# lucidrains/progen

Hardware: NVIDIA H100
Metric: tokens_per_sec (higher is better)
Workload: dtype bf16

## Files before the change

### progen_b200/csrc/gemm_tc.cu

```cuda
#include <cuda.h>
#include <mutex>
#include <unordered_map>
#include "gemm.h"
#include "tc_ptx.cuh"

namespace {

using namespace tc;

constexpr int BM = 128;
constexpr int BN = 128;
constexpr int BK = 64;
constexpr int WG_K = 16;
constexpr int THREADS = 384;
constexpr int A_BYTES = BM * BK * 2;
constexpr int B_BYTES = BN * BK * 2;
constexpr int STAGE_BYTES = A_BYTES + B_BYTES;
constexpr int STAGES = 6;
constexpr int CS_LD = BN + 4;
constexpr int SMEM_TOTAL = 1024  + STAGES * STAGE_BYTES + 2 * STAGES * 8;
static_assert(BM * CS_LD * 4 <= STAGES * STAGE_BYTES, "the epilogue tile reuses the operand ring");
static_assert(SMEM_TOTAL <= 227 * 1024, "H100: 227 KiB of shared memory per block");

struct GemmDev {
  int M, N, K;
  int batch, batch_reduce;
  int a_batch_rows, b_batch_rows;
  long long d_batch_rows;
  int causal, split_k;
  EpiArgs epi;
};

struct TileInfo {
  int z, m0, n0, kb_begin, kb_end;
};

__device__ __forceinline__ void decode_tile(const GemmDev& g, int t, TileInfo& ti) {
  const int m_tiles = (g.M + BM - 1) / BM;
  const int n_tiles = (g.N + BN - 1) / BN;
  const int per_z = g.split_k * m_tiles * n_tiles;
  ti.z = t / per_z;
  int r = t - ti.z * per_z;
  const int ks = r / (m_tiles * n_tiles);
  r -= ks * (m_tiles * n_tiles);
  ti.m0 = (r / n_tiles) * BM;
  ti.n0 = (r % n_tiles) * BN;
  const int kb_total = (g.K + BK - 1) / BK;
  int b = 0, e = kb_total;
  if (g.causal == 1) e = min(kb_total, (ti.m0 + BM + BK - 1) / BK);
  if (g.causal == 2) b = min(kb_total, ti.m0 / BK);
  if (g.split_k > 1) {
    const int per = (kb_total + g.split_k - 1) / g.split_k;
    b = min(kb_total, ks * per);
    e = min(kb_total, b + per);
  }
  ti.kb_begin = b;
  ti.kb_end = e;
}

template <bool A_MN, bool B_MN, int KIND, typename TO>
__global__ void __launch_bounds__(THREADS, 1)
gemm_tc_kernel(const __grid_constant__ CUtensorMap tma_a, const __grid_constant__ CUtensorMap tma_b, const GemmDev g) {
  extern __shared__ uint8_t smem_raw[];
  const uint32_t raw_u32 = smem_u32(smem_raw);
  const uint32_t smem_base = (raw_u32 + 1023u) & ~1023u;
  const uint32_t bar_base = smem_base + STAGES * STAGE_BYTES;
  auto full_bar = [&](int s) { return bar_base + 8u * s; };
  auto empty_bar = [&](int s) { return bar_base + 8u * (STAGES + s); };

  const int wg = threadIdx.x >> 7;
  TileInfo ti;
  decode_tile(g, blockIdx.x, ti);

  if (threadIdx.x == 0) {
    prefetch_tensormap(&tma_a);
    prefetch_tensormap(&tma_b);
    for (int s = 0; s < STAGES; ++s) {
      mbar_init(full_bar(s), 1);
      mbar_init(empty_bar(s), 2);
    }
    fence_barrier_init();
  }
  __syncthreads();

  if (wg == 0) {
    if (threadIdx.x == 0) {
      const int a_row0 = ti.z * g.a_batch_rows;
      const int b_row0 = ti.z * g.b_batch_rows;
      int stage = 0;
      uint32_t phase = 0;
      for (int kb = ti.kb_begin; kb < ti.kb_end; ++kb) {
        mbar_wait(empty_bar(stage), phase ^ 1);
        const uint32_t sa = smem_base + stage * STAGE_BYTES;
        const uint32_t sb = sa + A_BYTES;
        mbar_expect_tx(full_bar(stage), STAGE_BYTES);
        const int k0 = kb * BK;
        if constexpr (!A_MN) {
          tma_load_2d(sa, &tma_a, full_bar(stage), k0, a_row0 + ti.m0);
        } else {
#pragma unroll
          for (int i = 0; i < BM / 64; ++i)
            tma_load_2d(sa + i * 8192, &tma_a, full_bar(stage), ti.m0 + 64 * i, a_row0 + k0);
        }
        if constexpr (!B_MN) {
          tma_load_2d(sb, &tma_b, full_bar(stage), k0, b_row0 + ti.n0);
        } else {
#pragma unroll
          for (int i = 0; i < BN / 64; ++i)
            tma_load_2d(sb + i * 8192, &tma_b, full_bar(stage), ti.n0 + 64 * i, b_row0 + k0);
        }
        if (++stage == STAGES) { stage = 0; phase ^= 1; }
      }
    }
    return;
  }

  const int c = wg - 1;
  const int t = threadIdx.x - 128;
  float acc[64];
#pragma unroll
  for (int i = 0; i < 64; ++i) acc[i] = 0.f;
  {
    int stage = 0, prev = -1;
    uint32_t phase = 0;
    for (int kb = ti.kb_begin; kb < ti.kb_end; ++kb) {
      mbar_wait(full_bar(stage), phase);
      const uint32_t sa = smem_base + stage * STAGE_BYTES;
      const uint64_t adesc = make_smem_desc<A_MN>(sa + c * 8192);
      const uint64_t bdesc = make_smem_desc<B_MN>(sa + A_BYTES);
      constexpr uint32_t a_step = A_MN ? (2048 >> 4) : (32 >> 4), b_step = B_MN ? (2048 >> 4) : (32 >> 4);
      fence_regs(acc);
      wgmma_fence();
#pragma unroll
      for (int k = 0; k < BK / WG_K; ++k)
        wgmma_m64n128k16_bf16<A_MN ? 1 : 0, B_MN ? 1 : 0>(acc, adesc + (uint64_t)(k * a_step), bdesc + (uint64_t)(k * b_step));
      wgmma_commit();
      fence_regs(acc);
      wgmma_wait<1>();
      if (prev >= 0 && (t & 127) == 0) mbar_arrive(empty_bar(prev));
      prev = stage;
      if (++stage == STAGES) { stage = 0; phase ^= 1; }
    }
    wgmma_wait<0>();
    fence_regs(acc);
  }

  asm volatile("bar.sync 1, 256;" ::: "memory");
  float* cs = reinterpret_cast<float*>(smem_raw + (smem_base - raw_u32));
  {
    const int w = (t & 127) >> 5, lane = t & 31;
    const int r0 = 64 * c + 16 * w + (lane >> 2);
    const int c0 = 2 * (lane & 3);
#pragma unroll
    for (int j = 0; j < BN / 8; ++j) {
      *reinterpret_cast<float2*>(cs + r0 * CS_LD + 8 * j + c0) = make_float2(acc[4 * j], acc[4 * j + 1]);
      *reinterpret_cast<float2*>(cs + (r0 + 8) * CS_LD + 8 * j + c0) = make_float2(acc[4 * j + 2], acc[4 * j + 3]);
    }
  }
  asm volatile("bar.sync 1, 256;" ::: "memory");

#pragma unroll 1
  for (int idx = t; idx < BM * (BN / 8); idx += 256) {
    const int r = idx / (BN / 8), cc = (idx % (BN / 8)) * 8;
    const int m = ti.m0 + r, col = ti.n0 + cc;
    if (m >= g.M || col >= g.N) continue;
    float v[8];
    const float4 x0 = *reinterpret_cast<const float4*>(cs + r * CS_LD + cc);
    const float4 x1 = *reinterpret_cast<const float4*>(cs + r * CS_LD + cc + 4);
    v[0] = x0.x; v[1] = x0.y; v[2] = x0.z; v[3] = x0.w; v[4] = x1.x; v[5] = x1.y; v[6] = x1.z; v[7] = x1.w;
    const long long row = (g.batch_reduce ? 0 : (long long)ti.z * g.d_batch_rows) + m;
    epi_apply<KIND, TO, 8>(g.epi, DirectIO{}, row, col, v, true);
  }
}

typedef CUresult (*EncodeTiledFn)(CUtensorMap*, CUtensorMapDataType, cuuint32_t, void*, const cuuint64_t*,
                                  const cuuint64_t*, const cuuint32_t*, const cuuint32_t*, CUtensorMapInterleave,
                                  CUtensorMapSwizzle, CUtensorMapL2promotion, CUtensorMapFloatOOBfill);

EncodeTiledFn get_encode_fn() {
  static EncodeTiledFn fn = nullptr;
  static std::once_flag once;
  std::call_once(once, [] {
    void* p = nullptr;
    cudaDriverEntryPointQueryResult q;
    if (cudaGetDriverEntryPoint("cuTensorMapEncodeTiled", &p, cudaEnableDefault, &q) == cudaSuccess &&
        q == cudaDriverEntryPointSuccess)
      fn = reinterpret_cast<EncodeTiledFn>(p);
  });
  return fn;
}

struct MapKey {
  const void* ptr; uint64_t inner, outer, stride; uint32_t box_inner, box_outer, elem_bytes, swizzle;
  bool operator==(const MapKey& o) const {
    return ptr == o.ptr && inner == o.inner && outer == o.outer && stride == o.stride && box_inner == o.box_inner &&
           box_outer == o.box_outer && elem_bytes == o.elem_bytes && swizzle == o.swizzle;
  }
};
struct MapKeyHash {
  size_t operator()(const MapKey& k) const {
    size_t h = std::hash<const void*>()(k.ptr);
    auto mix = [&](uint64_t v) { h ^= std::hash<uint64_t>()(v) + 0x9e3779b97f4a7c15ULL + (h << 6) + (h >> 2); };
    mix(k.inner); mix(k.outer); mix(k.stride); mix(k.box_inner); mix(k.box_outer); mix(k.elem_bytes * 256 + k.swizzle);
    return h;
  }
};

int get_tensor_map(const void* ptr, uint64_t inner, uint64_t outer, uint64_t row_stride_elems, uint32_t box_inner,
                   uint32_t box_outer, CUtensorMap* out, uint32_t elem_bytes = 2, uint32_t swizzle = 128) {
  static std::unordered_map<MapKey, CUtensorMap, MapKeyHash> cache;
  static std::mutex mu;
  MapKey key{ptr, inner, outer, row_stride_elems, box_inner, box_outer, elem_bytes, swizzle};
  std::lock_guard<std::mutex> lock(mu);
  auto it = cache.find(key);
  if (it != cache.end()) { *out = it->second; return PROGEN_OK; }
  EncodeTiledFn fn = get_encode_fn();
  if (!fn) { progen_set_error("cuTensorMapEncodeTiled driver entry point not found"); return PROGEN_ERR_DEVICE; }
  cuuint64_t dims[2] = {inner, outer};
  cuuint64_t strides[1] = {row_stride_elems * elem_bytes};
  const CUtensorMapSwizzle sw = swizzle == 128 ? CU_TENSOR_MAP_SWIZZLE_128B : swizzle == 64 ? CU_TENSOR_MAP_SWIZZLE_64B
                              : swizzle == 32 ? CU_TENSOR_MAP_SWIZZLE_32B : CU_TENSOR_MAP_SWIZZLE_NONE;
  cuuint32_t box[2] = {box_inner, box_outer};
  cuuint32_t estr[2] = {1, 1};
  CUtensorMap m;
  CUresult r = fn(&m, elem_bytes == 4 ? CU_TENSOR_MAP_DATA_TYPE_FLOAT32 : CU_TENSOR_MAP_DATA_TYPE_BFLOAT16, 2,
                  const_cast<void*>(ptr), dims, strides, box, estr, CU_TENSOR_MAP_INTERLEAVE_NONE, sw, CU_TENSOR_MAP_L2_PROMOTION_L2_256B,
                  CU_TENSOR_MAP_FLOAT_OOB_FILL_NONE);
  if (r != CUDA_SUCCESS) {
    progen_set_error("cuTensorMapEncodeTiled failed (CUresult %d) ptr=%p inner=%llu outer=%llu stride=%llu box=%ux%u", (int)r,
                     ptr, (unsigned long long)inner, (unsigned long long)outer, (unsigned long long)row_stride_elems,
                     box_inner, box_outer);
    return PROGEN_ERR_CUDA;
  }
  if (cache.size() > 4096) cache.clear();
  cache.emplace(key, m);
  *out = m;
  return PROGEN_OK;
}


template <bool A_MN, bool B_MN, int KIND, typename TO>
int launch_inst(const CUtensorMap& ta, const CUtensorMap& tb, const GemmDev& gd, int tiles, cudaStream_t stream) {
  auto kern = gemm_tc_kernel<A_MN, B_MN, KIND, TO>;
  static bool attr_set = false;
  if (!attr_set) {
    PG_CUDA(cudaFuncSetAttribute(kern, cudaFuncAttributeMaxDynamicSharedMemorySize, SMEM_TOTAL));
    attr_set = true;
  }
  kern<<<tiles, THREADS, SMEM_TOTAL, stream>>>(ta, tb, gd);
  PG_LAUNCH_CHECK();
  return PROGEN_OK;
}

}

int pg_tensor_map_2d_bf16(const void* ptr, uint64_t inner, uint64_t outer, uint64_t row_stride_elems, uint32_t box_inner,
                          uint32_t box_outer, CUtensorMap* out) {
  return get_tensor_map(ptr, inner, outer, row_stride_elems, box_inner, box_outer, out);
}

int gemm_tc_launch(const GemmArgs& a, cudaStream_t stream) {
  PG_CHECK_ARG(a.in_dtype == PG_BF16);
  PG_CHECK_ARG(a.M > 0 && a.N > 0 && a.K > 0 && a.batch >= 1 && a.split_k >= 1);
  PG_CHECK_ARG(a.N % 32 == 0);
  PG_CHECK_ARG(a.K % BK == 0);
  PG_CHECK_ARG(a.lda % 8 == 0 && a.ldb % 8 == 0);
  PG_CHECK_ARG((reinterpret_cast<uintptr_t>(a.A) & 15) == 0 && (reinterpret_cast<uintptr_t>(a.B) & 15) == 0);
  PG_CHECK_ARG(!(a.split_k > 1 && a.causal));
  if (a.epi_kind == EPI_ROTARY) PG_CHECK_ARG(a.epi.seq_len % 32 == 0);
  PG_CHECK_ARG(!(a.split_k > 1 || a.batch_reduce) || (a.epi_kind == EPI_ACCUM && a.epi.atomic));

  const uint64_t a_rows = (a.batch > 1 && a.a_batch_rows > 0) ? (uint64_t)a.a_batch_rows * a.batch
                                                              : (uint64_t)(a.a_mn_major ? a.K : a.M);
  const uint64_t b_rows = (a.batch > 1 && a.b_batch_rows > 0) ? (uint64_t)a.b_batch_rows * a.batch
                                                              : (uint64_t)(a.b_mn_major ? a.K : a.N);
  CUtensorMap ta, tb;
  int rc;
  if (!a.a_mn_major) rc = get_tensor_map(a.A, a.K, a_rows, a.lda, BK, BM, &ta);
  else               rc = get_tensor_map(a.A, a.M, a_rows, a.lda, 64, BK, &ta);
  if (rc) return rc;
  if (!a.b_mn_major) rc = get_tensor_map(a.B, a.K, b_rows, a.ldb, BK, BN, &tb);
  else               rc = get_tensor_map(a.B, a.N, b_rows, a.ldb, 64, BK, &tb);
  if (rc) return rc;

  GemmDev gd;
  gd.M = a.M; gd.N = a.N; gd.K = a.K;
  gd.batch = a.batch; gd.batch_reduce = a.batch_reduce;
  gd.a_batch_rows = (int)a.a_batch_rows; gd.b_batch_rows = (int)a.b_batch_rows; gd.d_batch_rows = a.d_batch_rows;
  gd.causal = a.causal; gd.split_k = a.split_k;
  gd.epi = a.epi;
  const long long tiles = (long long)a.batch * a.split_k * ((a.M + BM - 1) / BM) * ((a.N + BN - 1) / BN);
  PG_CHECK_ARG(tiles < (1ll << 31));

  const int am = a.a_mn_major ? 1 : 0, bm = a.b_mn_major ? 1 : 0;
  const bool obf = a.out_dtype == PG_BF16;
#define TC_CASE(AM, BMJ, KIND, TO) return launch_inst<AM, BMJ, KIND, TO>(ta, tb, gd, (int)tiles, stream)
  switch (a.epi_kind) {
    case EPI_STORE:
      if (!am && bm) { if (obf) TC_CASE(false, true, EPI_STORE, bf16); else TC_CASE(false, true, EPI_STORE, float); }
      if (!am && !bm) { if (obf) TC_CASE(false, false, EPI_STORE, bf16); else TC_CASE(false, false, EPI_STORE, float); }
      if (am && bm) { if (obf) TC_CASE(true, true, EPI_STORE, bf16); else TC_CASE(true, true, EPI_STORE, float); }
      break;
    case EPI_ROTARY:
      if (!am && bm && obf) TC_CASE(false, true, EPI_ROTARY, bf16);
      break;
    case EPI_RESIDUAL:
      if (!am && bm) TC_CASE(false, true, EPI_RESIDUAL, float);
      break;
    case EPI_GLU:
      if (!am && bm && obf) TC_CASE(false, true, EPI_GLU, bf16);
      break;
    case EPI_GELU:
      if (!am && bm && obf) TC_CASE(false, true, EPI_GELU, bf16);
      break;
    case EPI_GLU_BWD:
      if (!am && !bm && obf) TC_CASE(false, false, EPI_GLU_BWD, bf16);
      break;
    case EPI_GELU_BWD:
      if (!am && !bm && obf) TC_CASE(false, false, EPI_GELU_BWD, bf16);
      break;
    case EPI_ACCUM:
      if (am && bm) TC_CASE(true, true, EPI_ACCUM, float);
      if (!am && !bm) TC_CASE(false, false, EPI_ACCUM, float);
      break;
    default: break;
  }
#undef TC_CASE
  progen_set_error("gemm_tc: unsupported combination epi=%d a_mn=%d b_mn=%d out=%d", a.epi_kind, am, bm, a.out_dtype);
  return PROGEN_ERR_UNSUPPORTED;
}
```

Baseline: 680,400.

## Make TC GEMM persistent with ping-pong consumer warpgroups and register reallocation

Turns the GEMM kernel into a persistent kernel launched on at most one block per SM. Each block walks tiles with a grid stride, and the two consumer warpgroups alternate whole 128x128 tiles, handing the turn over through named barriers so one group's epilogue overlaps the other's mainloop. Each consumer now holds a full 128-row tile, which is two 64x128 accumulators, and setmaxnreg moves registers from the producer to the consumers. The pipeline drops from 6 to 4 stages to make room for per-warpgroup epilogue staging buffers, which shrinks prefetch depth, and tiles are statically scheduled, so load balance may suffer on small grids.

Result: faster. 726,200 (median of 6 runs) (+6.7%).

```diff
diff --git a/progen_b200/csrc/gemm_tc.cu b/progen_b200/csrc/gemm_tc.cu
--- a/progen_b200/csrc/gemm_tc.cu
+++ b/progen_b200/csrc/gemm_tc.cu
@@ -1,4 +1,5 @@
 #include <cuda.h>
+#include <algorithm>
 #include <mutex>
 #include <unordered_map>
 #include "gemm.h"
@@ -16,11 +17,20 @@
 constexpr int A_BYTES = BM * BK * 2;
 constexpr int B_BYTES = BN * BK * 2;
 constexpr int STAGE_BYTES = A_BYTES + B_BYTES;
-constexpr int STAGES = 6;
+constexpr int STAGES = 4;
+constexpr int EPI_ROWS = 64;
 constexpr int CS_LD = BN + 4;
-constexpr int SMEM_TOTAL = 1024  + STAGES * STAGE_BYTES + 2 * STAGES * 8;
-static_assert(BM * CS_LD * 4 <= STAGES * STAGE_BYTES, "the epilogue tile reuses the operand ring");
+constexpr int CS_BYTES = EPI_ROWS * CS_LD * 4;
+constexpr int SMEM_TOTAL = 1024  + STAGES * STAGE_BYTES + 2 * CS_BYTES + 2 * STAGES * 8;
 static_assert(SMEM_TOTAL <= 227 * 1024, "H100: 227 KiB of shared memory per block");
+constexpr int BAR_TURN = 1, BAR_EPI = 3;
+constexpr int PRODUCER_REGS = 40, CONSUMER_REGS = 232;
+static_assert(128 * PRODUCER_REGS + 256 * CONSUMER_REGS <= 65536, "register file");
+
+__device__ __forceinline__ void named_bar_sync(int id, int n) { asm volatile("bar.sync %0, %1;" ::"r"(id), "r"(n) : "memory"); }
+__device__ __forceinline__ void named_bar_arrive(int id, int n) { asm volatile("bar.arrive %0, %1;" ::"r"(id), "r"(n) : "memory"); }
+template <int R> __device__ __forceinline__ void setmaxnreg_dec() { asm volatile("setmaxnreg.dec.sync.aligned.u32 %0;" ::"n"(R)); }
+template <int R> __device__ __forceinline__ void setmaxnreg_inc() { asm volatile("setmaxnreg.inc.sync.aligned.u32 %0;" ::"n"(R)); }
 
 struct GemmDev {
   int M, N, K;
@@ -60,116 +70,139 @@
 
 template <bool A_MN, bool B_MN, int KIND, typename TO>
 __global__ void __launch_bounds__(THREADS, 1)
-gemm_tc_kernel(const __grid_constant__ CUtensorMap tma_a, const __grid_constant__ CUtensorMap tma_b, const GemmDev g) {
+gemm_tc_kernel(const __grid_constant__ CUtensorMap tma_a, const __grid_constant__ CUtensorMap tma_b, const GemmDev g,
+               const int tiles) {
   extern __shared__ uint8_t smem_raw[];
   const uint32_t raw_u32 = smem_u32(smem_raw);
   const uint32_t smem_base = (raw_u32 + 1023u) & ~1023u;
-  const uint32_t bar_base = smem_base + STAGES * STAGE_BYTES;
+  const uint32_t cs_base = smem_base + STAGES * STAGE_BYTES;
+  const uint32_t bar_base = cs_base + 2 * CS_BYTES;
   auto full_bar = [&](int s) { return bar_base + 8u * s; };
   auto empty_bar = [&](int s) { return bar_base + 8u * (STAGES + s); };
 
   const int wg = threadIdx.x >> 7;
-  TileInfo ti;
-  decode_tile(g, blockIdx.x, ti);
-
   if (threadIdx.x == 0) {
     prefetch_tensormap(&tma_a);
     prefetch_tensormap(&tma_b);
     for (int s = 0; s < STAGES; ++s) {
       mbar_init(full_bar(s), 1);
-      mbar_init(empty_bar(s), 2);
+      mbar_init(empty_bar(s), 1);
     }
     fence_barrier_init();
   }
   __syncthreads();
 
+  int stage = 0;
+  uint32_t phase = 0;
+  auto advance = [&](int n) {
+    stage += n;
+    phase ^= (uint32_t)(stage / STAGES) & 1u;
+    stage %= STAGES;
+  };
+
   if (wg == 0) {
+    setmaxnreg_dec<PRODUCER_REGS>();
     if (threadIdx.x == 0) {
-      const int a_row0 = ti.z * g.a_batch_rows;
-      const int b_row0 = ti.z * g.b_batch_rows;
-      int stage = 0;
-      uint32_t phase = 0;
-      for (int kb = ti.kb_begin; kb < ti.kb_end; ++kb) {
-        mbar_wait(empty_bar(stage), phase ^ 1);
-        const uint32_t sa = smem_base + stage * STAGE_BYTES;
-        const uint32_t sb = sa + A_BYTES;
-        mbar_expect_tx(full_bar(stage), STAGE_BYTES);
-        const int k0 = kb * BK;
-        if constexpr (!A_MN) {
-          tma_load_2d(sa, &tma_a, full_bar(stage), k0, a_row0 + ti.m0);
-        } else {
-#pragma unroll
-          for (int i = 0; i < BM / 64; ++i)
-            tma_load_2d(sa + i * 8192, &tma_a, full_bar(stage), ti.m0 + 64 * i, a_row0 + k0);
+      for (int t = blockIdx.x; t < tiles; t += gridDim.x) {
+        TileInfo ti;
+        decode_tile(g, t, ti);
+        const int a_row0 = ti.z * g.a_batch_rows;
+        const int b_row0 = ti.z * g.b_batch_rows;
+        for (int kb = ti.kb_begin; kb < ti.kb_end; ++kb) {
+          mbar_wait(empty_bar(stage), phase ^ 1);
+          const uint32_t sa = smem_base + stage * STAGE_BYTES;
+          const uint32_t sb = sa + A_BYTES;
+          mbar_expect_tx(full_bar(stage), STAGE_BYTES);
+          const int k0 = kb * BK;
+          if constexpr (!A_MN) {
+            tma_load_2d(sa, &tma_a, full_bar(stage), k0, a_row0 + ti.m0);
+          } else {
+#pragma unroll
+            for (int i = 0; i < BM / 64; ++i)
+              tma_load_2d(sa + i * 8192, &tma_a, full_bar(stage), ti.m0 + 64 * i, a_row0 + k0);
+          }
+          if constexpr (!B_MN) {
+            tma_load_2d(sb, &tma_b, full_bar(stage), k0, b_row0 + ti.n0);
+          } else {
+#pragma unroll
+            for (int i = 0; i < BN / 64; ++i)
+              tma_load_2d(sb + i * 8192, &tma_b, full_bar(stage), ti.n0 + 64 * i, b_row0 + k0);
+          }
+          advance(1);
         }
-        if constexpr (!B_MN) {
-          tma_load_2d(sb, &tma_b, full_bar(stage), k0, b_row0 + ti.n0);
-        } else {
-#pragma unroll
-          for (int i = 0; i < BN / 64; ++i)
-            tma_load_2d(sb + i * 8192, &tma_b, full_bar(stage), ti.n0 + 64 * i, b_row0 + k0);
-        }
-        if (++stage == STAGES) { stage = 0; phase ^= 1; }
       }
     }
     return;
   }
 
+  setmaxnreg_inc<CONSUMER_REGS>();
   const int c = wg - 1;
-  const int t = threadIdx.x - 128;
-  float acc[64];
-#pragma unroll
-  for (int i = 0; i < 64; ++i) acc[i] = 0.f;
-  {
-    int stage = 0, prev = -1;
-    uint32_t phase = 0;
+  const int tid = threadIdx.x & 127;
+  float* cs = reinterpret_cast<float*>(smem_raw + (cs_base - raw_u32)) + c * (CS_BYTES / 4);
+  for (int p = 0, t = blockIdx.x; t < tiles; ++p, t += gridDim.x) {
+    TileInfo ti;
+    decode_tile(g, t, ti);
+    if ((p & 1) != c) {
+      advance(ti.kb_end - ti.kb_begin);
+      continue;
+    }
+    float acc[2][64];
+#pragma unroll
+    for (int i = 0; i < 64; ++i) acc[0][i] = acc[1][i] = 0.f;
+    if (p > 0) named_bar_sync(BAR_TURN + c, 256);
+    int prev = -1;
     for (int kb = ti.kb_begin; kb < ti.kb_end; ++kb) {
       mbar_wait(full_bar(stage), phase);
       const uint32_t sa = smem_base + stage * STAGE_BYTES;
-      const uint64_t adesc = make_smem_desc<A_MN>(sa + c * 8192);
+      const uint64_t adesc0 = make_smem_desc<A_MN>(sa), adesc1 = make_smem_desc<A_MN>(sa + 8192);
       const uint64_t bdesc = make_smem_desc<B_MN>(sa + A_BYTES);
       constexpr uint32_t a_step = A_MN ? (2048 >> 4) : (32 >> 4), b_step = B_MN ? (2048 >> 4) : (32 >> 4);
-      fence_regs(acc);
+      fence_regs(acc[0]);
+      fence_regs(acc[1]);
       wgmma_fence();
 #pragma unroll
-      for (int k = 0; k < BK / WG_K; ++k)
-        wgmma_m64n128k16_bf16<A_MN ? 1 : 0, B_MN ? 1 : 0>(acc, adesc + (uint64_t)(k * a_step), bdesc + (uint64_t)(k * b_step));
+      for (int k = 0; k < BK / WG_K; ++k) {
+        wgmma_m64n128k16_bf16<A_MN ? 1 : 0, B_MN ? 1 : 0>(acc[0], adesc0 + (uint64_t)(k * a_step), bdesc + (uint64_t)(k * b_step));
+        wgmma_m64n128k16_bf16<A_MN ? 1 : 0, B_MN ? 1 : 0>(acc[1], adesc1 + (uint64_t)(k * a_step), bdesc + (uint64_t)(k * b_step));
+      }
       wgmma_commit();
-      fence_regs(acc);
+      fence_regs(acc[0]);
+      fence_regs(acc[1]);
       wgmma_wait<1>();
-      if (prev >= 0 && (t & 127) == 0) mbar_arrive(empty_bar(prev));
+      if (prev >= 0 && tid == 0) mbar_arrive(empty_bar(prev));
       prev = stage;
-      if (++stage == STAGES) { stage = 0; phase ^= 1; }
-    }
+      advance(1);
+    }
+    if (t + (int)gridDim.x < tiles) named_bar_arrive(BAR_TURN + (c ^ 1), 256);
     wgmma_wait<0>();
-    fence_regs(acc);
-  }
-
-  asm volatile("bar.sync 1, 256;" ::: "memory");
-  float* cs = reinterpret_cast<float*>(smem_raw + (smem_base - raw_u32));
-  {
-    const int w = (t & 127) >> 5, lane = t & 31;
-    const int r0 = 64 * c + 16 * w + (lane >> 2);
-    const int c0 = 2 * (lane & 3);
-#pragma unroll
-    for (int j = 0; j < BN / 8; ++j) {
-      *reinterpret_cast<float2*>(cs + r0 * CS_LD + 8 * j + c0) = make_float2(acc[4 * j], acc[4 * j + 1]);
-      *reinterpret_cast<float2*>(cs + (r0 + 8) * CS_LD + 8 * j + c0) = make_float2(acc[4 * j + 2], acc[4 * j + 3]);
-    }
-  }
-  asm volatile("bar.sync 1, 256;" ::: "memory");
-
+    fence_regs(acc[0]);
+    fence_regs(acc[1]);
+    if (prev >= 0 && tid == 0) mbar_arrive(empty_bar(prev));
+
+    const int w = tid >> 5, lane = tid & 31;
+    const int r0 = 16 * w + (lane >> 2), c0 = 2 * (lane & 3);
+#pragma unroll
+    for (int h = 0; h < 2; ++h) {
+      named_bar_sync(BAR_EPI + c, 128);
+#pragma unroll
+      for (int j = 0; j < BN / 8; ++j) {
+        *reinterpret_cast<float2*>(cs + r0 * CS_LD + 8 * j + c0) = make_float2(acc[h][4 * j], acc[h][4 * j + 1]);
+        *reinterpret_cast<float2*>(cs + (r0 + 8) * CS_LD + 8 * j + c0) = make_float2(acc[h][4 * j + 2], acc[h][4 * j + 3]);
+      }
+      named_bar_sync(BAR_EPI + c, 128);
 #pragma unroll 1
-  for (int idx = t; idx < BM * (BN / 8); idx += 256) {
-    const int r = idx / (BN / 8), cc = (idx % (BN / 8)) * 8;
-    const int m = ti.m0 + r, col = ti.n0 + cc;
-    if (m >= g.M || col >= g.N) continue;
-    float v[8];
-    const float4 x0 = *reinterpret_cast<const float4*>(cs + r * CS_LD + cc);
-    const float4 x1 = *reinterpret_cast<const float4*>(cs + r * CS_LD + cc + 4);
-    v[0] = x0.x; v[1] = x0.y; v[2] = x0.z; v[3] = x0.w; v[4] = x1.x; v[5] = x1.y; v[6] = x1.z; v[7] = x1.w;
-    const long long row = (g.batch_reduce ? 0 : (long long)ti.z * g.d_batch_rows) + m;
-    epi_apply<KIND, TO, 8>(g.epi, DirectIO{}, row, col, v, true);
+      for (int idx = tid; idx < EPI_ROWS * (BN / 8); idx += 128) {
+        const int r = idx / (BN / 8), cc = (idx % (BN / 8)) * 8;
+        const int m = ti.m0 + EPI_ROWS * h + r, col = ti.n0 + cc;
+        if (m >= g.M || col >= g.N) continue;
+        float v[8];
+        const float4 x0 = *reinterpret_cast<const float4*>(cs + r * CS_LD + cc);
+        const float4 x1 = *reinterpret_cast<const float4*>(cs + r * CS_LD + cc + 4);
+        v[0] = x0.x; v[1] = x0.y; v[2] = x0.z; v[3] = x0.w; v[4] = x1.x; v[5] = x1.y; v[6] = x1.z; v[7] = x1.w;
+        const long long row = (g.batch_reduce ? 0 : (long long)ti.z * g.d_batch_rows) + m;
+        epi_apply<KIND, TO, 8>(g.epi, DirectIO{}, row, col, v, true);
+      }
+    }
   }
 }
 
@@ -247,7 +280,7 @@
     PG_CUDA(cudaFuncSetAttribute(kern, cudaFuncAttributeMaxDynamicSharedMemorySize, SMEM_TOTAL));
     attr_set = true;
   }
-  kern<<<tiles, THREADS, SMEM_TOTAL, stream>>>(ta, tb, gd);
+  kern<<<std::min(tiles, pg_num_sms()), THREADS, SMEM_TOTAL, stream>>>(ta, tb, gd, tiles);
   PG_LAUNCH_CHECK();
   return PROGEN_OK;
 }
```
